# KevinLADLee/RoboRTS-Edu-SLAM

Hardware: AMD Instinct MI355X
Metric: candidate-pose scorings/sec (1081-beam scan, 2000×2000 grid) at 1/2/4/8 GPUs (higher is better)
Workload: dtype f64; 1 GPU; config2: 1081-beam scans vs 2000x2000 @5cm fp32 grid, full 3-level coarse->fine->super-fine (sim-YAML windows 5070+1331+189 candidates/scan); levels=headline, scans_per_gpu=4096, parallelism=replicas x1 (scan-sharded, no collective)

## Files before the change

roborts-edu-slam_amd/csrc/csm_api.cpp:

```cpp
#include "csm_source_digest.h"
#include "csm_host.hpp"
#include "libm_sincos.hpp"

using namespace csmh;

extern "C" {

int csm_abi_version(void) { return CSM_ABI_VERSION; }

const char* csm_build_digest(void) { return CSM_SOURCE_DIGEST; }

int csm_create(int device, csm_ctx** out) {
  const char* lr = std::getenv("LOCAL_RANK");
  const char* lw = std::getenv("LOCAL_WORLD_SIZE");
  const int world = lw ? std::max(1, std::atoi(lw)) : 1;
  const int rank = (lr && world > 1) ? std::min(std::max(0, std::atoi(lr)), world - 1) : 0;
  return create_context(device, rank, world, out);
}

int csm_get_host_plan(csm_ctx* c, csm_host_plan* out) {
  if (!c || !out) return CSM_ERR_INVALID_ARG;
  *out = c->host_plan;
  return CSM_OK;
}
// ... 17 lines not shown
    return CSM_ERR_HIP;
  }
  context_host_plan(device, local_rank, local_world, &c->host_plan);
  if (const char* env = std::getenv("CSM_HOST_THREADS")) {
    const int v = std::atoi(env);
    if (v > 0) c->host_plan.threads = v;
  }
  c->host_threads = c->host_plan.threads;
  if (const char* env = std::getenv("CSM_FIRST_WINDOWS")) c->first_windows = c->first_windows_submit = std::max(0, std::atoi(env));
  if (const char* env = std::getenv("CSM_FIRST_WINDOWS_SUBMIT")) c->first_windows_submit = std::max(0, std::atoi(env));
  if (const char* env = std::getenv("CSM_SPLIT_HANDOFF_MIN")) c->split_handoff_min = std::max(2, std::atoi(env));
  if (const char* env = std::getenv("CSM_DEFER_HANDOFF")) c->defer_last_handoff = std::atoi(env) != 0;
  if (const char* env = std::getenv("CSM_HOST_SIGNAL")) c->host_signal = std::atoi(env) != 0;
  if (const char* env = std::getenv("CSM_FINISH")) {
    c->device_finish = std::strcmp(env, "host") != 0;
    c->fast_finish = std::strcmp(env, "exact") != 0;
  }
  if (const char* env = std::getenv("CSM_KERNEL")) {
    c->row_kernel = std::strcmp(env, "v2") != 0;
    c->box_kernel = std::strcmp(env, "v6") == 0 || std::strcmp(env, "v7") == 0;
    c->box_kernel = c->box_kernel || std::strcmp(env, "v8") == 0;
    c->phase_kernel = std::strcmp(env, "v7") == 0 || std::strcmp(env, "v8") == 0;
    c->tiny_kernel = std::strcmp(env, "v8") == 0;
    c->pair_kernel = false;
  }
  if (const char* env = std::getenv("CSM_PHASE_STRIPS")) c->phase_strips = std::atoi(env) != 0;
  if (const char* env = std::getenv("CSM_BG_RUNS")) c->bg_runs = std::max(0, std::min(std::atoi(env), 3));
  if (const char* env = std::getenv("CSM_PHASE_MARGIN_LOG2"))
    c->phase_margin_log2 = std::max(2, std::min(std::atoi(env), 20));
  if (const char* env = std::getenv("CSM_PIPELINE")) {
    const int v = std::atoi(env);
    c->pipeline_min = v > 0 ? v : INT32_MAX;
  }
  if (const char* env = std::getenv("CSM_PIPELINE_PARTS"))
    c->pipeline_parts = std::max(2, std::min(std::atoi(env), csm_ctx::kMaxParts));
  if (const char* env = std::getenv("CSM_SKIP_DEAD_LISTS")) c->skip_dead_lists = std::atoi(env) != 0;
  if (const char* env = std::getenv("CSM_SMALL")) c->small_path = std::atoi(env) != 0;
  if (const char* env = std::getenv("CSM_LIST_REDUCE_MIN")) c->list_reduce_min = std::max<long long>(0, std::atoll(env));
  if (const char* env = std::getenv("CSM_STATS_DUMP")) c->stats_dump = std::atoi(env) != 0;
  if (const char* env = std::getenv("CSM_SCORE_MARKER")) c->score_marker = std::atoi(env) != 0;
  if (const char* env = std::getenv("CSM_DEVICE_TRIG")) c->device_trig = std::atoi(env) != 0;
#ifdef CSM_DEBUG_FIN
  c->debug_fin = true;
#endif
  if (c->each_slot([](LaunchSlot& s) { return s.create_sync_events(); }) != hipSuccess ||
      c->ev_pts.create(hipEventDisableTiming) != hipSuccess || c->ev_pack.create(hipEventDisableTiming) != hipSuccess ||
      c->x_stream.create(hipStreamNonBlocking) != hipSuccess) {
    delete c;
    return CSM_ERR_HIP;
  }
  {
    hipError_t we = c->h_pts.ensure((size_t)64 << 10);
    if (we == hipSuccess) we = c->pts.ensure((size_t)64 << 10);
    for (hipStream_t st : std::initializer_list<hipStream_t>{c->stream, c->h2d, c->d2h}) {
      if (we != hipSuccess) break;
      std::memset(c->h_pts.p, 0, (size_t)64 << 10);
      we = hipMemcpyAsync(c->pts.p, c->h_pts.p, (size_t)64 << 10, hipMemcpyHostToDevice, st);
      if (we == hipSuccess) we = hipMemcpyAsync(c->h_pts.p, c->pts.p, (size_t)64 << 10, hipMemcpyDeviceToHost, st);
      if (we == hipSuccess) we = hipStreamSynchronize(st);
    }
    if (we != hipSuccess) {
      csm_destroy(c);
      return CSM_ERR_HIP;
    }
  }
  *out = c;
  if (c->stats_dump) csm_set_profiling(c, 1);
  return CSM_OK;
// ... 251 lines not shown
```

roborts-edu-slam_amd/csrc/csm_driver.cpp:

```cpp
#include "csm_driver_internal.hpp"

using namespace csmh;

namespace {

struct BorrowedBatch {
  csm_ctx* c;
  ScanBatch* b;
  BorrowedBatch(csm_ctx* cc, ScanBatch* bb) : c(cc), b(bb) {
    if (b) c->swap_batch(*b);
  }
  ~BorrowedBatch() {
    if (b) c->swap_batch(*b);
  }
  BorrowedBatch(const BorrowedBatch&) = delete;
  BorrowedBatch& operator=(const BorrowedBatch&) = delete;
};

}

int csmh::matchers_loaded_locked(csm_ctx* c, const csm_param all_levels[3], int32_t use_fine, double* poses,
                                 double* covs, double* scores, int32_t first_level, const double* score_seed) {
  if (c->n_scans < 0) return c->fail(CSM_ERR_INVALID_ARG, "no scans loaded (csm_load_scans)");
  if (!c->has_grid) return c->fail(CSM_ERR_NO_GRID, "no grid set");
  const int32_t n_scans = c->n_scans;
  if (n_scans == 0) return CSM_OK;
  const double t_call = now_ms();
  c->t_call = t_call;
  if (c->profiling && c->t_exit > 0.0) c->account("host:between_calls", (float)(t_call - c->t_exit), 0.0, 0.0);
  std::vector<double> resp((size_t)n_scans, 0.0), sum((size_t)n_scans, 0.0);
  if (score_seed) sum.assign(score_seed, score_seed + n_scans);
  const csm_param* levels = all_levels + first_level;
  const int n_levels = use_fine ? 3 - first_level : 1;
// ... 46 lines not shown
  return match_level(c, n_scans, off.data(), *param, poses, covs, responses, argmax_flat);
}

int csm_scan_match(csm_ctx* c, const double* pts, int32_t n_points, const csm_param* param,
                   double pose[3], double cov[9], double* response, int64_t* argmax_flat) {
  if (!c || !response) return CSM_ERR_INVALID_ARG;
  const int64_t off[2] = {0, n_points < 0 ? 0 : n_points};
  if (n_points < 0) return c->fail(CSM_ERR_INVALID_ARG, "negative point count");
  return csm_scan_match_batch(c, 1, pts, off, param, pose, cov, response, argmax_flat);
}

int csm_scan_matchers_submit(csm_ctx* c, const csm_param levels[3], int32_t use_fine, double* poses, double* covs,
                             double* scores) {
  if (!c || !levels || !poses || !covs || !scores) return CSM_ERR_INVALID_ARG;
  std::lock_guard<std::mutex> lk(c->mu);
  DeviceGuard g(c->device);
  int st;
  if (c->staged_count == 0 && c->n_scans < 0) return c->fail(CSM_ERR_INVALID_ARG, "no scans loaded (csm_load_scans)");
  if (!c->has_grid) return c->fail(CSM_ERR_NO_GRID, "no grid set");
  ScanBatch* parked = nullptr;
  if (c->staged_count > 0) {
    parked = &c->staged[c->staged_head].batch;
    if ((st = take_staged(c)) != CSM_OK) return st;
  }
  auto prior_last_launches = [&]() {
    BorrowedBatch own(c, parked);
    return pipe_last_launches(c);
  };
  const int32_t n_scans = c->n_scans;
  const int n_levels = use_fine ? 3 : 1;
  bool fast = false;
  for (int l = 0; l < n_levels; ++l) fast |= levels[l].type == CSM_FAST;
  const int32_t* grid = c->scan_grid.empty() ? nullptr : c->scan_grid.data();
  const int K = std::max(2, std::min(c->pipeline_parts, csm_ctx::kMaxParts));
  if (n_scans == 0 || fast || grid || n_scans < c->pipeline_min || 2 * K > csm_ctx::kMaxParts) {
    if ((st = prior_last_launches()) != CSM_OK || (st = pipe_drain(c)) != CSM_OK) return st;
    return matchers_loaded_locked(c, levels, use_fine, poses, covs, scores);
  }
  const double t_call = now_ms();
  c->t_call = t_call;
  PipeState& PS = pipe_of(c);
  PipeJob& J = PS.job[PS.next];
  PipeJob& P = PS.job[PS.next ^ 1];
  if (J.pending && ((st = prior_last_launches()) != CSM_OK || (st = pipe_drain(c)) != CSM_OK))
    return st;
  PipeMode mode(c);
  job_setup(c, J, n_scans, c->scan_off.data(), levels, n_levels, poses, covs, nullptr, nullptr, K, PS.next * K,
            true);
  J.own_sum.assign((size_t)n_scans, 0.0);
  J.sum = J.own_sum.data();
  J.scores = scores;
  if ((st = job_begin(c, J, 0)) != CSM_OK) return pipe_abort(c, st);
  if ((st = prior_last_launches()) != CSM_OK) return pipe_abort(c, st);
  for (int h = 1; h < K; ++h)
    if ((st = job_begin(c, J, h)) != CSM_OK) return pipe_abort(c, st);
  if (P.pending && (st = job_finish(c, P)) != CSM_OK) return pipe_abort(c, st);
  if ((st = job_levels(c, J)) != CSM_OK) return pipe_abort(c, st);
  PS.next ^= 1;
  if (c->profiling) {
    c->t_exit = now_ms();
    c->account("host:submit", (float)(c->t_exit - t_call), 0.0, 0.0);
  }
  return CSM_OK;
}

int csm_scan_matchers_wait(csm_ctx* c) {
  if (!c) return CSM_ERR_INVALID_ARG;
  std::lock_guard<std::mutex> lk(c->mu);
  DeviceGuard g(c->device);
  return pipe_drain(c);
}

int csm_scan_matchers_loaded(csm_ctx* c, const csm_param levels[3], int32_t use_fine, double* poses,
                             double* covs, double* scores) {
  if (!c || !levels || !poses || !covs || !scores) return CSM_ERR_INVALID_ARG;
  std::lock_guard<std::mutex> lk(c->mu);
  DeviceGuard g(c->device);
  int st0;
  if ((st0 = pipe_drain(c)) != CSM_OK || (st0 = take_staged(c)) != CSM_OK) return st0;
  return matchers_loaded_locked(c, levels, use_fine, poses, covs, scores);
}

int csm_scan_matchers_batch(csm_ctx* c, int32_t n_scans, const double* pts, const int64_t* offsets,
                            const csm_param levels[3], int32_t use_fine, double* poses, double* covs,
                            double* scores) {
  if (!c || !levels || !poses || !covs || !scores) return CSM_ERR_INVALID_ARG;
  std::lock_guard<std::mutex> lk(c->mu);
  DeviceGuard g(c->device);
  const int st = load_scans_locked(c, n_scans, pts, offsets);
  if (st != CSM_OK) return st;
// ... 40 lines not shown
```

roborts-edu-slam_amd/csrc/csm_driver_internal.hpp:

```cpp
#pragma once

#include "csm_host.hpp"

namespace csmh {

struct LevelRun {
  csm_param P{};
  Dims D;
  std::vector<int> scan_of;
  std::vector<WindowPlan> plans;
  std::vector<int64_t> pt_off;
  std::vector<int32_t> grid;
  const AngleEntry* angles = nullptr;
  AngleEntry* rows = nullptr;
  const csm::FinishOut* fin = nullptr;
  const double* scores = nullptr;
  bool dev = false;
  int skip_lists = 0;
  PendingRun pend;
  int tag = -1;
  std::vector<csm::FinishOut>* snap = nullptr;
  std::vector<char>* how = nullptr;
  mutable int err = 0;
  const int32_t* order = nullptr;
// ... 26 lines not shown
    sw = nullptr;
    sw_stride = 0;
    int_bad = 0;
    int_known = false;
    shape = LevelSummary{};
    range_preset = false;
    dev_trig = false;
    trig_bad = 0;
  }
};

struct PipeJob {
  int K = 2, n_levels = 0, slot0 = 0;
  int first_windows = 0;
  int32_t n_scans = 0;
  const int64_t* offsets = nullptr;
  const int32_t* scan_grid = nullptr;
  csm_param levels[3]{};
  double *poses = nullptr, *covs = nullptr, *sum = nullptr;
  double* scores = nullptr;
  std::vector<double> resp, own_sum;
  int32_t first[csm_ctx::kMaxParts]{}, count[csm_ctx::kMaxParts]{};
  LevelRun R[2][csm_ctx::kMaxParts];
  bool pending = false;
  bool last_handoff_done = false;
  std::vector<int32_t> order[csm_ctx::kMaxParts];
  std::vector<csm::FinishOut> snaps[csm_ctx::kMaxParts];
  std::vector<char> hows[csm_ctx::kMaxParts];
};

struct PipeState {
  PipeJob job[2];
  int next = 0;
};

struct PipeMode {
  csm_ctx* c;
  bool small_was;
  explicit PipeMode(csm_ctx* cc) : c(cc), small_was(cc->small_path) {
    c->small_path = false;
    c->early_now = true;
  }
  ~PipeMode() {
    c->small_path = small_was;
    c->early_now = false;
  }
};

int live_lists(const csm_param* levels, int n_levels, int l);
int level_begin(csm_ctx* c, int32_t n_scans, const int64_t* offsets, const csm_param& P, const double* poses,
                double* responses, int64_t* argmax_flat, LevelRun& R, const int32_t* scan_grid, int skip_lists);
int level_begin_split(csm_ctx* c, int32_t n_scans, const int64_t* offsets, const csm_param& P, const double* poses,
                      double* responses, LevelRun& R, const int32_t* scan_grid, int skip_lists, int first);
int level_end(csm_ctx* c, LevelRun& R, double* poses, double* covs, double* responses, int64_t* argmax_flat);
int level_end_begin(csm_ctx* c, LevelRun& R, LevelRun& N, int32_t n_scans, const int64_t* offsets,
                    const csm_param& P, double* poses, double* covs, double* responses, double* sum,
                    const int32_t* scan_grid, int skip_lists, bool split = false);

PipeState& pipe_of(csm_ctx* c);
void job_setup(csm_ctx* c, PipeJob& J, int32_t n_scans, const int64_t* offsets, const csm_param* levels,
               int n_levels, double* poses, double* covs, double* sum, const int32_t* scan_grid, int K, int slot0,
               bool submitted = false);
int job_begin(csm_ctx* c, PipeJob& J, int h);
int job_levels(csm_ctx* c, PipeJob& J);
int job_finish(csm_ctx* c, PipeJob& J);
int pipe_abort(csm_ctx* c, int st);
int pipe_last_launches(csm_ctx* c);
int match_levels_pipelined(csm_ctx* c, int32_t n_scans, const int64_t* offsets, const csm_param* levels,
                           int n_levels, double* poses, double* covs, double* sum,
                           const int32_t* scan_grid = nullptr);

}
```

roborts-edu-slam_amd/csrc/csm_host.hpp:

```cpp
#pragma once

#include "csm.h"
#include "csm_internal.hpp"
#include "csm_finish_rules.hpp"
#include "csm_gridmap.h"
#include "csm_gridmap_internal.hpp"
#include "csm_resources.hpp"
#include "host_math.hpp"
#include "csm_pyramid.hpp"
#include "csm_search_match.hpp"
#include "csm_level_decision.hpp"
#include "csm_grid_copies.hpp"

#include <algorithm>
#include <atomic>
#include <chrono>
#include <condition_variable>
#include <functional>
#include <memory>
#include <cfloat>
#include <cmath>
#include <cstdio>
#include <cstdlib>
#include <cstring>
// ... 214 lines not shown
    }
  }
  int n_threads_;
  csm_host_plan plan_;
  static constexpr int chunk_div_ = 8;
  std::vector<std::thread> workers_;
  std::mutex mu_;
  std::condition_variable cv_;
  const std::function<void(int)>* job_ = nullptr;
  int n_items_ = 0, wanted_ = 0, chunk_ = 1;
  std::atomic<uint64_t> epoch_{0};
  std::atomic<uint64_t> claim_{0};
  std::atomic<int> done_{0};
  bool stop_ = false;
  int64_t start_ns_ = 0;
  std::atomic<int64_t> first_join_ns_{0}, last_join_ns_{0}, busy_ns_{0};
  double last_caller_share_ = 0.0, last_join_us_ = -1.0, last_last_join_us_ = -1.0, last_wall_us_ = 0.0,
         last_busy_us_ = 0.0;
};

inline double now_ms() {
  return std::chrono::duration<double, std::milli>(std::chrono::steady_clock::now().time_since_epoch()).count();
}


struct PendingRun {
  char kname[48] = {0};
  char fname[48] = {0};
  double alg_bytes = 0.0, scorings = 0.0, finish_bytes = 0.0;
  bool device_finish = false, timed = false;
  hipEvent_t ev0 = nullptr, ev1 = nullptr, ev2 = nullptr, done = nullptr;
  hipEvent_t ev_fast = nullptr;
  hipEvent_t gap0 = nullptr, gap1 = nullptr;
  const int32_t* flags = nullptr;
  int n_flags = 0;
  const csm::FinishOut* fin_host = nullptr;
  const int32_t* host_flag = nullptr;
  int32_t flag_value = 0;
  const int32_t* fast_flag = nullptr;
  bool defer_timing = false;
};

struct CtxStreams {
  Stream stream;
  Stream h2d, d2h;
  Stream x_stream;
  Stream stage_stream;
};

struct LaunchSlot {
  DevBuf scans, angles, scores, partials, best, fin;
  DevBuf ang_max;
  DevBuf win_ctr;
  HostBuf h_scores, h_fin, h_angles, h_sw;
  HostBuf h_angles_next;
  DevBuf fin_sig;
  HostBuf h_fin_sig;
  Event ev0, ev1, ev2;
  Event ev_ft;
  Event ev_g0, ev_g1;
  Event ev_done;
  Event ev_in;
  Event ev_k;
  Event ev_fast;
  bool span_gap = false;
  int32_t list_tag = 0;
  bool tail_open = false;

  hipError_t create_sync_events() {
    hipError_t e = hipSuccess;
    for (Event* ev : {&ev_done, &ev_in, &ev_k, &ev_fast})
      if (e == hipSuccess) e = ev->create(hipEventDisableTiming);
    return e;
  }
  hipError_t create_timing_events() {
    hipError_t e = hipSuccess;
    for (Event* ev : {&ev0, &ev1, &ev2, &ev_ft, &ev_g0, &ev_g1})
      if (e == hipSuccess) e = ev->create(hipEventDefault);
    return e;
  }
};

struct GridState {
  csm_map_info info{};
  bool has_grid = false;
  const float* d_grid = nullptr;
  DevBuf grid_buf;
  DevBuf gridi;
  const int32_t* d_gridi = nullptr;
  const void* key_cells = nullptr;
  int64_t key_stride = 0, key_version = -1;
  int32_t key_sx = -1, key_sy = -1;
  bool int_checked = false, int_ok = false;
  int int_exp = 0;
  int32_t pitch = 0;
  int32_t n_grids = 1;
  int32_t outside_i = 0;
  double int_max_abs = 0.0;
// ... 117 lines not shown
  Staged staged[2];
  int staged_head = 0, staged_count = 0;
  void swap_batch(csmh::ScanBatch& b) {
    std::swap(static_cast<csmh::ScanBatch&>(*this), b);
    pts_cached = b.pts_cached = false;
  }
  csmh::DevBuf laser_tab;
  bool laser_tab_ready = false;
  int32_t laser_tab_beams = 0;
  uint32_t laser_tab_amin = 0, laser_tab_ainc = 0;
  csmh::DevBuf deskew_tab;
  std::vector<double> deskew_tab_host;
  bool deskew_tab_ready = false;
  int32_t deskew_tab_beams = 0;
  uint32_t deskew_tab_amin = 0, deskew_tab_ainc = 0;

  bool profiling = false;
  bool profile_first_level = false;
  bool stats_dump = false;

  static constexpr int kMaxParts = 4;
  csmh::LaunchSlot alt[kMaxParts - 1];
  template <class F>
  hipError_t each_slot(F&& fn) {
    hipError_t e = fn(static_cast<csmh::LaunchSlot&>(*this));
    for (auto& a : alt)
      if (e == hipSuccess) e = fn(a);
    return e;
  }
  int pipeline_min = 512;
  bool skip_dead_lists = true;
  int64_t list_reduce_min = 8192;
  int pipeline_parts = 2;
  int first_windows = 128;
  int first_windows_submit = 512;
  int first_windows_submit_min_use = 512;
  int span_growth = 4;
  void* pipe = nullptr;
  bool split_last_handoff = true;
  int split_handoff_min = 256;
  bool defer_last_handoff = true;
  int part0_permille = 550;
  int part0_permille_submit = 500;
  void swap_slot(int i) {
    std::swap(static_cast<csmh::LaunchSlot&>(*this), alt[i - 1]);
  }
  void account_pool(const char* what) {
    if (!profiling || !pool) return;
    char nm[48];
    std::snprintf(nm, sizeof(nm), "pool:%s", what);
    account(nm, (float)(std::max(0.0, pool->last_join_us()) * 1e-3), pool->last_caller_share(), 0.0);
    std::snprintf(nm, sizeof(nm), "pool:%s:wall", what);
    account(nm, (float)(pool->last_wall_us() * 1e-3), std::max(0.0, pool->last_last_join_us()), pool->last_busy_us());
  }
  std::vector<csmh::PendingRun> deferred;
  std::vector<csm_kernel_stat> stats;
  void account_count(const char* name, int64_t n) {
    account(name, 0.0f, 0.0, 0.0);
    for (auto& s : stats)
      if (std::strncmp(s.name, name, sizeof(s.name)) == 0) s.launches += n - 1;
  }
  void account(const char* name, float ms, double bytes, double scorings) {
    for (auto& s : stats)
      if (std::strncmp(s.name, name, sizeof(s.name)) == 0) {
        s.launches += 1;
        s.total_ms += ms;
// ... 138 lines not shown
```

roborts-edu-slam_amd/csrc/csm_launch.cpp:

```cpp
#include "csm_host.hpp"
#include "libm_sincos_table.hpp"

namespace csmh {

int window_dims(const csm_param& P, Dims& d) {
  if (!(P.search_angle_resolution > 0.0) || !(P.search_space_resolution > 0.0) ||
      !(P.search_angle_offset >= 0.0) || !(P.search_space_size >= 0.0))
    return CSM_ERR_INVALID_ARG;
  const double half = (P.search_angle_offset * 2) / 2;
  const double na = std::floor(half * 2 / P.search_angle_resolution) + 1;
  const double ns = round_half_away(P.search_space_size / P.search_space_resolution) + 1;
  if (!(na >= 1.0 && na < 1e7 && ns >= 1.0 && ns < 1e7)) return CSM_ERR_INVALID_ARG;
  d.n_angles = (int32_t)na;
  d.n_space = (int32_t)ns;
  d.n_cand = (int64_t)d.n_angles * d.n_space * d.n_space;
  return CSM_OK;
}

bool beam_rule(int n, int use_point_size, int& step, int& use, int& n_used) {
  use = use_point_size;
  if (n < 2 * use) {
    use = n;
    step = 1;
  } else {
// ... 34 lines not shown
    }
    if (p.timed && (e = hipEventSynchronize(p.done)) != hipSuccess) return c->hip_fail(e, "hipEventSynchronize");
  } else if ((e = hipEventSynchronize(p.done)) != hipSuccess) {
    return c->hip_fail(e, "hipEventSynchronize");
  }
  return account_run(c, p);
}

int flush_deferred(csm_ctx* c) {
  int st = CSM_OK;
  for (const PendingRun& p : c->deferred) {
    const hipError_t e = hipEventSynchronize(p.done);
    if (e != hipSuccess) {
      st = c->hip_fail(e, "hipEventSynchronize(deferred)");
      break;
    }
    if ((st = account_run(c, p)) != CSM_OK) break;
  }
  c->deferred.clear();
  return st;
}

int account_run(csm_ctx* c, const PendingRun& p) {
  hipError_t e;
  if (p.timed) {
    float ms = 0.f;
    if ((e = hipEventElapsedTime(&ms, p.ev0, p.ev1)) != hipSuccess) return c->hip_fail(e, "hipEventElapsedTime");
    if (p.gap0) {
      float g = 0.f;
      if ((e = hipEventElapsedTime(&g, p.gap0, p.gap1)) != hipSuccess) return c->hip_fail(e, "hipEventElapsedTime");
      ms -= g;
    }
    c->account(p.kname, ms, p.alg_bytes, p.scorings);
    if (p.gap0) {
      char nm[48];
      std::snprintf(nm, sizeof(nm), "span2:%.41s", p.kname);
      c->account(nm, ms, p.alg_bytes, 0.0);
    }
    if (p.device_finish) {
      if ((e = hipEventElapsedTime(&ms, p.ev1, p.ev2)) != hipSuccess) return c->hip_fail(e, "hipEventElapsedTime");
      c->account(p.fname, ms, p.finish_bytes, 0.0);
      if (p.ev_fast) {
        float mf = 0.f, mx = 0.f;
        if ((e = hipEventElapsedTime(&mf, p.ev1, p.ev_fast)) != hipSuccess ||
            (e = hipEventElapsedTime(&mx, p.ev_fast, p.ev2)) != hipSuccess)
          return c->hip_fail(e, "hipEventElapsedTime");
        const char* lt = std::strchr(p.fname, '<');
        char nm[48];
        std::snprintf(nm, sizeof(nm), "finish:fast%s", lt ? lt : "");
        c->account(nm, mf, 0.0, 0.0);
        std::snprintf(nm, sizeof(nm), "finish:exact%s", lt ? lt : "");
        c->account(nm, mx, 0.0, 0.0);
      }
      if (p.flags) {
        int exact = 0;
        for (int i = 0; i < p.n_flags; ++i) exact += p.flags[i] != 0;
        c->account("finish:exact_windows", 0.f, 0.0, (double)exact);
        char nm[48];
        const char* lt = std::strchr(p.fname, '<');
        std::snprintf(nm, sizeof(nm), "finish:exact_windows%s", lt ? lt : "");
        c->account(nm, 0.f, (double)p.n_flags, (double)exact);
      }
    }
  }
  return CSM_OK;
}

bool phase_table(double f, int ns, int margin_log2, csm::PhaseTable& T) {
  T = csm::PhaseTable{};
  if (!(f > 0.0 && f < 1.0) || ns < 1 || ns > csm::kPhaseMaxSpace) return false;
// ... 493 lines not shown
    case ScoreKernel::kBoxPair:
      return csm::launch_score_box_pair(L, d_sw, d_pts, d_ang, d_out, d_partials, s.n_space, stream);
    case ScoreKernel::kBox: return csm::launch_score_box(L, d_sw, d_pts, d_ang, d_out, d_partials, s.n_space, stream);
    case ScoreKernel::kBoxTiled: return csm::launch_score_box(L, d_sw, d_pts, d_ang, d_out, d_partials, 16, stream);
    case ScoreKernel::kPhase:
      return csm::launch_score_phase(L, PT, d_sw, d_pts, d_ang, d_out, d_partials, s.n_space, stream);
    case ScoreKernel::kTiny: return csm::launch_score_tiny(L, d_sw, d_pts, d_ang, d_out, d_partials, s.n_space, stream);
    case ScoreKernel::kRows:
      return csm::launch_score_rows(L, d_sw, d_pts, d_ang, d_out, d_partials, s.n_space, s.rows_sq, stream);
    case ScoreKernel::kCols: return csm::launch_score_cols(L, d_sw, d_pts, d_ang, d_out, d_partials, s.kt, stream);
  }
  return hipErrorInvalidValue;
}

int Launch::scoring() {
  const bool best = mode == Finish::kBest;
  hipError_t e;
  if (sp.score && c->score_marker && !(c->profiling && w0 == 0) &&
      (e = hipEventRecord(c->ev_k, c->stream)) != hipSuccess)
    return c->hip_fail(e, "hipEventRecord");
  if (c->profiling && sp.score && w0 == 0 && (e = hipEventRecord(c->ev0, c->stream)) != hipSuccess)
    return c->hip_fail(e, "hipEventRecord");
  if (c->profiling && sp.score && w0 > 0 && !c->span_gap) {
    if ((e = hipEventRecord(c->ev_g1, c->stream)) != hipSuccess) return c->hip_fail(e, "hipEventRecord");
    c->span_gap = true;
  }
  if (best) {
    if ((e = c->partials.ensure((size_t)nw * (size_t)shape.bps * sizeof(BestPartial))) != hipSuccess)
      return c->hip_fail(e, "hipMalloc(partials)");
    if ((e = c->best.ensure((size_t)nw * sizeof(BestPartial))) != hipSuccess) return c->hip_fail(e, "hipMalloc(best)");
  } else if ((e = c->scores.ensure((size_t)nw * (size_t)stride * sizeof(double))) != hipSuccess) {
    return c->hip_fail(e, "hipMalloc(scores)");
  }
  if (sp.score &&
      (e = launch_score(shape, L, PT, (const ScanWork*)c->scans.p + w0, (const double*)c->pts.p,
                        (const AngleEntry*)c->angles.p, best ? nullptr : (double*)c->scores.p,
                        best ? (BestPartial*)c->partials.p : nullptr, c->stream)) != hipSuccess)
    return c->hip_fail(e, best ? "score kernel (best)" : "score kernel");
  if (dec.tail && sp.score) c->tail_open = w1 < nw;
  if (sp.score && c->profiling && (e = hipEventRecord(c->ev1, c->stream)) != hipSuccess)
    return c->hip_fail(e, "hipEventRecord");
  if (sp.score && !sp.finish && w0 == 0 && c->profiling && (e = hipEventRecord(c->ev_g0, c->stream)) != hipSuccess)
    return c->hip_fail(e, "hipEventRecord");
  return CSM_OK;
}

int Launch::finish_scores_to_host() {
  const size_t bytes = (size_t)nw * (size_t)D.n_cand * sizeof(double);
  hipError_t e;
  if ((e = c->h_scores.ensure(bytes)) != hipSuccess) return c->hip_fail(e, "hipHostMalloc(scores)");
  if ((e = hipEventRecord(c->ev_k, c->stream)) != hipSuccess || (e = hipStreamWaitEvent(c->d2h, c->ev_k, 0)) != hipSuccess)
    return c->hip_fail(e, "kernels event");
  if ((e = hipMemcpyAsync(c->h_scores.p, c->scores.p, bytes, hipMemcpyDeviceToHost, c->d2h)) != hipSuccess)
    return c->hip_fail(e, "hipMemcpyAsync(scores)");
  return CSM_OK;
}

int Launch::launch_finish_timed(const csm::FinishArgs& A, csm::FinishOut* out, hipStream_t fs, bool fast_done) {
  hipError_t e;
  if ((e = csm::launch_finish(A, (const ScanWork*)c->scans.p, (const AngleEntry*)c->angles.p,
                              (const double*)c->scores.p, out, nw, c->stream, fs, c->ev_fast, fast_done)) != hipSuccess)
    return c->hip_fail(e, "finish_kernel");
  if (time_fin() && fs != c->stream && (e = hipEventRecord(c->ev_ft, c->stream)) != hipSuccess)
    return c->hip_fail(e, "hipEventRecord");
  if (time_fin() && (e = hipEventRecord(c->ev2, fs)) != hipSuccess) return c->hip_fail(e, "hipEventRecord");
  return CSM_OK;
// ... 34 lines not shown
  const BestPartial* parts = (const BestPartial*)c->partials.p;
  hipError_t e;
  if (shape.kernel == ScoreKernel::kBoxTiled) {
    const int32_t tpw = shape.ktiles * shape.ktiles;
    if ((e = c->best_tiles.ensure((size_t)nw * tpw * sizeof(BestPartial))) != hipSuccess)
      return c->hip_fail(e, "hipMalloc(tile bests)");
    if ((e = csm::launch_reduce_best(parts, D.n_angles, nw * tpw, (BestPartial*)c->best_tiles.p, c->stream)) !=
            hipSuccess ||
        (e = csm::launch_reduce_best((const BestPartial*)c->best_tiles.p, tpw, nw, (BestPartial*)c->best.p,
                                     c->stream)) != hipSuccess)
      return c->hip_fail(e, "reduce_best_kernel");
  } else if ((e = csm::launch_reduce_best(parts, (int32_t)shape.bps, nw, (BestPartial*)c->best.p, c->stream)) !=
             hipSuccess) {
    return c->hip_fail(e, "reduce_best_kernel");
  }
  if ((e = hipEventRecord(c->ev_k, c->stream)) != hipSuccess || (e = hipStreamWaitEvent(c->d2h, c->ev_k, 0)) != hipSuccess)
    return c->hip_fail(e, "kernels event");
  if ((e = hipMemcpyAsync(best_out, c->best.p, (size_t)nw * sizeof(BestPartial), hipMemcpyDeviceToHost, c->d2h)) != hipSuccess)
    return c->hip_fail(e, "hipMemcpyAsync(best)");
  return CSM_OK;
}

void Launch::fill_pending(const char* kname, PendingRun& p) {
  pending_base(c, D, plans, kname, p);
  p.flags = flags_h;
  p.n_flags = n_flags;
  p.device_finish = mode == Finish::kDevice && time_fin();
  p.ev_fast = (time_fin() && mode == Finish::kDevice && c->fast_finish && c->x_stream) ? (hipEvent_t)c->ev_ft : nullptr;
  if (c->span_gap) {
    p.gap0 = c->ev_g0;
    p.gap1 = c->ev_g1;
    c->span_gap = false;
  }
  p.fin_host = sig_out;
  p.host_flag = SA.host_flag;
  p.fast_flag = SA.host_fast_flag;
  p.flag_value = SA.flag_value;
  p.defer_timing = sig;
}

int run_windows(csm_ctx* c, const csm_param& P, const Dims& D, const Geometry& G,
                const std::vector<WindowPlan>& plans, const std::vector<int64_t>& pt_offsets,
                const AngleEntry* angles, size_t n_angle_entries,
                const std::vector<int32_t>& grid_index, BestPartial* best_out,
                Finish mode, PendingRun* pend, int skip_lists, WinSpan sp) {
  if (best_out) mode = Finish::kBest;
  const int nw = (int)plans.size();
  if (nw == 0) return CSM_OK;
  const int w0 = sp.w1 < 0 ? 0 : sp.w0, w1 = sp.w1 < 0 ? nw : sp.w1;
  Launch X{c,  P,  D,  G,  plans, angles, n_angle_entries, mode, skip_lists,
           sp, nw, w0, w1, w0 == 0 && w1 == nw && sp.score && sp.finish, P.search_space_resolution / G.mres};
  const double tp0 = c->profiling ? now_ms() : 0.0;
  if (!c->deferred.empty()) {
    const int fst = flush_deferred(c);
    if (fst != CSM_OK) return fst;
  }
  const double tp1 = c->profiling ? now_ms() : 0.0;
  if (c->profiling) c->account("host:launch:flush_events", (float)(tp1 - tp0), 0.0, 0.0);
  int st;
  hipError_t e;
  if ((st = X.validate()) != CSM_OK) return st;
  if (X.whole && mode != Finish::kBest && c->int_ok && X.S.in_range && small_launch(c, D, nw))
    return run_windows_small(c, P, D, G, plans, pt_offsets, angles, n_angle_entries, grid_index,
                             mode == Finish::kDevice, pend, skip_lists);
  if ((st = X.decide()) != CSM_OK) return st;
  if ((st = X.level_work(pt_offsets, grid_index)) != CSM_OK) return st;
// ... 156 lines not shown
```

roborts-edu-slam_amd/csrc/csm_pipeline.cpp:

```cpp
#include "csm_driver_internal.hpp"

namespace csmh {
namespace {

template <typename F>
int with_slot(csm_ctx* c, const PipeJob& J, int h, F&& f) {
  const int sidx = J.slot0 + h;
  if (sidx > 0) c->swap_slot(sidx);
  const int st = f();
  if (sidx > 0) c->swap_slot(sidx);
  return st;
}

#ifndef CSM_WINDOW_ORDER
#define CSM_WINDOW_ORDER 1
#endif
void window_order(const Geometry& G, const double* poses, int32_t n, std::vector<int32_t>& out) {
  out.resize((size_t)n);
  thread_local std::vector<uint32_t> key, key2;
  thread_local std::vector<int32_t> idx2;
  key.resize((size_t)n);
  key2.resize((size_t)n);
  idx2.resize((size_t)n);
  auto spread = [](uint32_t v) {
    v &= 0xFFFF;
    v = (v | (v << 8)) & 0x00FF00FFu;
    v = (v | (v << 4)) & 0x0F0F0F0Fu;
    v = (v | (v << 2)) & 0x33333333u;
    v = (v | (v << 1)) & 0x55555555u;
    return v;
  };
  for (int32_t s = 0; s < n; ++s) {
    double m[3];
    G.to_map(poses + 3 * (size_t)s, m);
    const double qx = std::floor(m[0] / 64.0), qy = std::floor(m[1] / 64.0);
    const uint32_t ix = (uint32_t)((int32_t)std::max(-32768.0, std::min(32767.0, qx)) + 32768);
    const uint32_t iy = (uint32_t)((int32_t)std::max(-32768.0, std::min(32767.0, qy)) + 32768);
    key[(size_t)s] = spread(ix) | (spread(iy) << 1);
  }
  std::vector<int32_t>& idx = out;
  for (int32_t s = 0; s < n; ++s) idx[(size_t)s] = s;
  for (int shift = 0; shift < 32; shift += 8) {
    size_t cnt[257] = {0};
    for (int32_t i = 0; i < n; ++i) ++cnt[((key[(size_t)i] >> shift) & 0xFF) + 1];
    for (int d = 0; d < 256; ++d) cnt[d + 1] += cnt[d];
    for (int32_t i = 0; i < n; ++i) {
      const size_t o = cnt[(key[(size_t)i] >> shift) & 0xFF]++;
      key2[o] = key[(size_t)i];
      idx2[o] = idx[(size_t)i];
    }
    key.swap(key2);
    idx.swap(idx2);
  }
  if (CSM_WINDOW_ORDER == 2) return;
  idx2.assign(idx.begin(), idx.end());
  int32_t pos = 0;
  for (int x = 0; x < 8; ++x)
    for (int32_t m = x; m < n; m += 8) out[(size_t)pos++] = idx2[(size_t)m];
}

int job_skip(const csm_ctx* c, const PipeJob& J, int l) {
  return c->skip_dead_lists ? live_lists(J.levels, J.n_levels, l) : 0;
}

int job_handoff(csm_ctx* c, PipeJob& J, int l, int h) {
  const int32_t s0 = J.first[h];
  J.R[(l + 1) & 1][h].tag = (l + 1) * 8 + h;
  const bool timed = c->profiling;
  c->profiling = timed && !c->profile_first_level;
  const int st = with_slot(c, J, h, [&] {
    return level_end_begin(c, J.R[l & 1][h], J.R[(l + 1) & 1][h], J.count[h], J.offsets + s0, J.levels[l + 1],
                           J.poses + 3 * (size_t)s0, J.covs + 9 * (size_t)s0, J.resp.data() + s0, J.sum + s0,
                           J.scan_grid ? J.scan_grid + s0 : nullptr, job_skip(c, J, l + 1),
                           c->split_last_handoff && h == J.K - 1 && l + 2 == J.n_levels);
  });
  c->profiling = timed;
  return st;
}

int job_last_handoff(csm_ctx* c, PipeJob& J) {
  if (!J.pending || J.last_handoff_done) return CSM_OK;
  J.last_handoff_done = true;
  return job_handoff(c, J, J.n_levels - 2, J.K - 1);
}

}

PipeState& pipe_of(csm_ctx* c) {
  if (!c->pipe) c->pipe = new PipeState();
  return *static_cast<PipeState*>(c->pipe);
}

void job_setup(csm_ctx* c, PipeJob& J, int32_t n_scans, const int64_t* offsets, const csm_param* levels,
               int n_levels, double* poses, double* covs, double* sum, const int32_t* scan_grid, int K, int slot0,
               bool submitted) {
  J.K = K;
  J.first_windows = !submitted ? c->first_windows
                    : (n_levels > 0 && levels[0].use_point_size > c->first_windows_submit_min_use) ? c->first_windows_submit
                                                                                                   : 0;
  const int permille = submitted ? c->part0_permille_submit : c->part0_permille;
  J.n_levels = n_levels;
  J.slot0 = slot0;
  J.n_scans = n_scans;
  J.offsets = offsets;
  J.scan_grid = scan_grid;
  for (int l = 0; l < n_levels; ++l) J.levels[l] = levels[l];
  J.poses = poses;
  J.covs = covs;
  J.sum = sum;
  J.scores = nullptr;
  J.pending = false;
  J.last_handoff_done = false;
  const int64_t n0 = (K == 2 && permille > 0) ? (int64_t)n_scans * permille / 1000
                                                        : (int64_t)n_scans / K;
  for (int h = 0; h < K; ++h) {
    J.first[h] = h == 0 ? 0 : (int32_t)(n0 + (int64_t)(n_scans - n0) * (h - 1) / (K - 1));
    J.count[h] = (h == 0 ? (int32_t)n0 : (int32_t)(n0 + (int64_t)(n_scans - n0) * h / (K - 1))) - J.first[h];
  }
  J.resp.assign((size_t)n_scans, 0.0);
  for (auto& row : J.R)
    for (LevelRun& r : row) r.reset();
  for (int h = 0; h < K; ++h) J.order[h].clear();
}

int job_begin(csm_ctx* c, PipeJob& J, int h) {
  const int32_t s0 = J.first[h];
  J.R[0][h].tag = h;
  if (CSM_WINDOW_ORDER) {
    window_order(Geometry(c->info), J.poses + 3 * (size_t)s0, J.count[h], J.order[h]);
    J.R[0][h].order = J.R[1][h].order = J.order[h].data();
  }
  return with_slot(c, J, h, [&] {
    const int32_t* g = J.scan_grid ? J.scan_grid + s0 : nullptr;
    if (h == 0)
      return level_begin_split(c, J.count[h], J.offsets + s0, J.levels[0], J.poses + 3 * (size_t)s0,
                               J.resp.data() + s0, J.R[0][h], g, job_skip(c, J, 0), J.first_windows);
    return level_begin(c, J.count[h], J.offsets + s0, J.levels[0], J.poses + 3 * (size_t)s0, J.resp.data() + s0,
                       nullptr, J.R[0][h], g, job_skip(c, J, 0));
  });
}

int job_levels(csm_ctx* c, PipeJob& J) {
  const int K = J.K, n_levels = J.n_levels;
  int st;
  for (int l = 0; l + 1 < n_levels; ++l)
    for (int h = 0; h < K; ++h) {
      if (c->defer_last_handoff && l + 2 == n_levels && h == K - 1) continue;
      if ((st = job_handoff(c, J, l, h)) != CSM_OK) return st;
    }
  J.pending = true;
  J.last_handoff_done = n_levels < 2 || !c->defer_last_handoff;
  return CSM_OK;
}

int job_finish(csm_ctx* c, PipeJob& J) {
  if (!J.pending) return CSM_OK;
  int st;
  if ((st = job_last_handoff(c, J)) != CSM_OK) return st;
  J.pending = false;
  const int K = J.K, last = J.n_levels - 1;
  for (int h = 0; h < K; ++h) {
    const int32_t s0 = J.first[h];
    LevelRun& cur = J.R[last & 1][h];
    if (c->debug_fin) {
      J.snaps[h].assign(cur.scan_of.size(), csm::FinishOut{});
      J.hows[h].assign(cur.scan_of.size(), (char)3);
      cur.snap = &J.snaps[h];
      cur.how = &J.hows[h];
    }
    if ((st = level_end(c, cur, J.poses + 3 * (size_t)s0, J.covs + 9 * (size_t)s0, J.resp.data() + s0, nullptr)) !=
        CSM_OK)
      return st;
    for (int s = s0; s < s0 + J.count[h]; ++s) J.sum[(size_t)s] += J.resp[(size_t)s];
  }
  if (J.scores)
    for (int s = 0; s < J.n_scans; ++s) J.scores[s] = J.sum[(size_t)s] / J.n_levels;
  if (c->debug_fin) {
    (void)hipDeviceSynchronize();
    for (int h = 0; h < K; ++h) {
      const LevelRun& L = J.R[last & 1][h];
      if (!L.dev || !L.fin) continue;
      for (size_t i = 0; i < J.snaps[h].size(); ++i) {
        const csm::FinishOut& a = J.snaps[h][i];
        const csm::FinishOut& b = L.fin[i];
        const int lists = (int)(b.seal_tag_kind >> 34) & 3;
// ... 73 lines not shown
```

Before: 13.89 billion scorings/s.

## Submit unsplit single-part job when coarse level is device-bound

Adds a submit-order planner that picks the number of pipeline parts per submitted job. When the coarse level is device-bound and no part count was set, it uses one part instead of two. With one part, the first handoff is issued before the prior job's finish to keep the device fed. Slot indexing now uses a fixed half-capacity, and the profiler records dispatch counts. The trade is fewer, larger launches and less intra-job overlap against lower per-part launch and sync overhead.

```diff
diff --git a/roborts-edu-slam_amd/csrc/csm_api.cpp b/roborts-edu-slam_amd/csrc/csm_api.cpp
--- a/roborts-edu-slam_amd/csrc/csm_api.cpp
+++ b/roborts-edu-slam_amd/csrc/csm_api.cpp
@@ -73,8 +73,12 @@
     const int v = std::atoi(env);
     c->pipeline_min = v > 0 ? v : INT32_MAX;
   }
-  if (const char* env = std::getenv("CSM_PIPELINE_PARTS"))
+  if (const char* env = std::getenv("CSM_PIPELINE_PARTS")) {
     c->pipeline_parts = std::max(2, std::min(std::atoi(env), csm_ctx::kMaxParts));
+    c->pipeline_parts_set = true;
+  }
+  if (const char* env = std::getenv("CSM_SUBMIT_PARTS")) c->submit_parts = std::max(0, std::min(std::atoi(env), 2));
+  if (const char* env = std::getenv("CSM_SINGLE_SPLIT_HANDOFF")) c->single_split_handoff = std::atoi(env) != 0;
   if (const char* env = std::getenv("CSM_SKIP_DEAD_LISTS")) c->skip_dead_lists = std::atoi(env) != 0;
   if (const char* env = std::getenv("CSM_SMALL")) c->small_path = std::atoi(env) != 0;
   if (const char* env = std::getenv("CSM_LIST_REDUCE_MIN")) c->list_reduce_min = std::max<long long>(0, std::atoll(env));
diff --git a/roborts-edu-slam_amd/csrc/csm_driver.cpp b/roborts-edu-slam_amd/csrc/csm_driver.cpp
--- a/roborts-edu-slam_amd/csrc/csm_driver.cpp
+++ b/roborts-edu-slam_amd/csrc/csm_driver.cpp
@@ -1,4 +1,5 @@
 #include "csm_driver_internal.hpp"
+#include "csm_submit_order.hpp"
 
 using namespace csmh;
 
@@ -111,8 +112,9 @@
   bool fast = false;
   for (int l = 0; l < n_levels; ++l) fast |= levels[l].type == CSM_FAST;
   const int32_t* grid = c->scan_grid.empty() ? nullptr : c->scan_grid.data();
-  const int K = std::max(2, std::min(c->pipeline_parts, csm_ctx::kMaxParts));
-  if (n_scans == 0 || fast || grid || n_scans < c->pipeline_min || 2 * K > csm_ctx::kMaxParts) {
+  const int K = submit_parts(c->submit_parts, c->pipeline_parts_set, std::min(c->pipeline_parts, csm_ctx::kMaxParts),
+                             coarse_device_bound(c, levels, n_levels));
+  if (n_scans == 0 || fast || grid || n_scans < c->pipeline_min || K > PipeState::kParts) {
     if ((st = prior_last_launches()) != CSM_OK || (st = pipe_drain(c)) != CSM_OK) return st;
     return matchers_loaded_locked(c, levels, use_fine, poses, covs, scores);
   }
@@ -124,17 +126,23 @@
   if (J.pending && ((st = prior_last_launches()) != CSM_OK || (st = pipe_drain(c)) != CSM_OK))
     return st;
   PipeMode mode(c);
-  job_setup(c, J, n_scans, c->scan_off.data(), levels, n_levels, poses, covs, nullptr, nullptr, K, PS.next * K,
-            true);
+  job_setup(c, J, n_scans, c->scan_off.data(), levels, n_levels, poses, covs, nullptr, nullptr, K,
+            PS.next * PipeState::kParts, true);
   J.own_sum.assign((size_t)n_scans, 0.0);
   J.sum = J.own_sum.data();
   J.scores = scores;
-  if ((st = job_begin(c, J, 0)) != CSM_OK) return pipe_abort(c, st);
-  if ((st = prior_last_launches()) != CSM_OK) return pipe_abort(c, st);
-  for (int h = 1; h < K; ++h)
-    if ((st = job_begin(c, J, h)) != CSM_OK) return pipe_abort(c, st);
-  if (P.pending && (st = job_finish(c, P)) != CSM_OK) return pipe_abort(c, st);
-  if ((st = job_levels(c, J)) != CSM_OK) return pipe_abort(c, st);
+  const SubmitOrder order = submit_order(K, P.pending ? P.K : 0, n_levels, c->defer_last_handoff);
+  for (int i = 0; i < order.n; ++i) {
+    const SubmitOp& op = order.op[i];
+    switch (op.step) {
+      case SubmitStep::kBegin: st = job_begin(c, J, op.part); break;
+      case SubmitStep::kHandoff: st = job_handoff(c, J, op.level, op.part); break;
+      case SubmitStep::kPriorLast: st = prior_last_launches(); break;
+      case SubmitStep::kPriorFinish: st = job_finish(c, P); break;
+    }
+    if (st != CSM_OK) return pipe_abort(c, st);
+  }
+  job_launched(c, J);
   PS.next ^= 1;
   if (c->profiling) {
     c->t_exit = now_ms();
diff --git a/roborts-edu-slam_amd/csrc/csm_driver_internal.hpp b/roborts-edu-slam_amd/csrc/csm_driver_internal.hpp
--- a/roborts-edu-slam_amd/csrc/csm_driver_internal.hpp
+++ b/roborts-edu-slam_amd/csrc/csm_driver_internal.hpp
@@ -82,6 +82,7 @@
 struct PipeState {
   PipeJob job[2];
   int next = 0;
+  static constexpr int kParts = csm_ctx::kMaxParts / 2;
 };
 
 struct PipeMode {
@@ -96,6 +97,10 @@
     c->early_now = false;
   }
 };
+
+inline bool coarse_device_bound(const csm_ctx* c, const csm_param* levels, int n_levels) {
+  return n_levels > 0 && levels[0].use_point_size > c->first_windows_submit_min_use;
+}
 
 int live_lists(const csm_param* levels, int n_levels, int l);
 int level_begin(csm_ctx* c, int32_t n_scans, const int64_t* offsets, const csm_param& P, const double* poses,
@@ -112,7 +117,9 @@
                int n_levels, double* poses, double* covs, double* sum, const int32_t* scan_grid, int K, int slot0,
                bool submitted = false);
 int job_begin(csm_ctx* c, PipeJob& J, int h);
+int job_handoff(csm_ctx* c, PipeJob& J, int l, int h);
 int job_levels(csm_ctx* c, PipeJob& J);
+void job_launched(const csm_ctx* c, PipeJob& J);
 int job_finish(csm_ctx* c, PipeJob& J);
 int pipe_abort(csm_ctx* c, int st);
 int pipe_last_launches(csm_ctx* c);
diff --git a/roborts-edu-slam_amd/csrc/csm_host.hpp b/roborts-edu-slam_amd/csrc/csm_host.hpp
--- a/roborts-edu-slam_amd/csrc/csm_host.hpp
+++ b/roborts-edu-slam_amd/csrc/csm_host.hpp
@@ -270,6 +270,7 @@
   hipEvent_t ev0 = nullptr, ev1 = nullptr, ev2 = nullptr, done = nullptr;
   hipEvent_t ev_fast = nullptr;
   hipEvent_t gap0 = nullptr, gap1 = nullptr;
+  int dispatches = 1;
   const int32_t* flags = nullptr;
   int n_flags = 0;
   const csm::FinishOut* fin_host = nullptr;
@@ -302,6 +303,7 @@
   Event ev_k;
   Event ev_fast;
   bool span_gap = false;
+  int span_count = 0;
   int32_t list_tag = 0;
   bool tail_open = false;
 
@@ -485,6 +487,9 @@
   bool skip_dead_lists = true;
   int64_t list_reduce_min = 8192;
   int pipeline_parts = 2;
+  bool pipeline_parts_set = false;
+  int submit_parts = 0;
+  bool single_split_handoff = false;
   int first_windows = 128;
   int first_windows_submit = 512;
   int first_windows_submit_min_use = 512;
diff --git a/roborts-edu-slam_amd/csrc/csm_launch.cpp b/roborts-edu-slam_amd/csrc/csm_launch.cpp
--- a/roborts-edu-slam_amd/csrc/csm_launch.cpp
+++ b/roborts-edu-slam_amd/csrc/csm_launch.cpp
@@ -90,10 +90,12 @@
       ms -= g;
     }
     c->account(p.kname, ms, p.alg_bytes, p.scorings);
+    if (p.dispatches > 1) c->account_count(p.kname, p.dispatches - 1);
     if (p.gap0) {
       char nm[48];
       std::snprintf(nm, sizeof(nm), "span2:%.41s", p.kname);
       c->account(nm, ms, p.alg_bytes, 0.0);
+      if (p.dispatches > 1) c->account_count(nm, p.dispatches - 1);
     }
     if (p.device_finish) {
       if ((e = hipEventElapsedTime(&ms, p.ev1, p.ev2)) != hipSuccess) return c->hip_fail(e, "hipEventElapsedTime");
@@ -653,6 +655,7 @@
   } else if ((e = c->scores.ensure((size_t)nw * (size_t)stride * sizeof(double))) != hipSuccess) {
     return c->hip_fail(e, "hipMalloc(scores)");
   }
+  if (sp.score) c->span_count = w0 == 0 ? 1 : c->span_count + 1;
   if (sp.score &&
       (e = launch_score(shape, L, PT, (const ScanWork*)c->scans.p + w0, (const double*)c->pts.p,
                         (const AngleEntry*)c->angles.p, best ? nullptr : (double*)c->scores.p,
@@ -753,6 +756,8 @@
     p.gap1 = c->ev_g1;
     c->span_gap = false;
   }
+  p.dispatches = std::max(1, c->span_count);
+  c->span_count = 0;
   p.fin_host = sig_out;
   p.host_flag = SA.host_flag;
   p.fast_flag = SA.host_fast_flag;
diff --git a/roborts-edu-slam_amd/csrc/csm_pipeline.cpp b/roborts-edu-slam_amd/csrc/csm_pipeline.cpp
--- a/roborts-edu-slam_amd/csrc/csm_pipeline.cpp
+++ b/roborts-edu-slam_amd/csrc/csm_pipeline.cpp
@@ -1,4 +1,5 @@
 #include "csm_driver_internal.hpp"
+#include "csm_submit_order.hpp"
 
 namespace csmh {
 namespace {
@@ -63,41 +64,40 @@
   return c->skip_dead_lists ? live_lists(J.levels, J.n_levels, l) : 0;
 }
 
+}
+
+PipeState& pipe_of(csm_ctx* c) {
+  if (!c->pipe) c->pipe = new PipeState();
+  return *static_cast<PipeState*>(c->pipe);
+}
+
 int job_handoff(csm_ctx* c, PipeJob& J, int l, int h) {
   const int32_t s0 = J.first[h];
   J.R[(l + 1) & 1][h].tag = (l + 1) * 8 + h;
   const bool timed = c->profiling;
   c->profiling = timed && !c->profile_first_level;
+  const bool split = (J.K > 1 ? c->split_last_handoff : c->single_split_handoff) && h == J.K - 1 && l + 2 == J.n_levels;
   const int st = with_slot(c, J, h, [&] {
     return level_end_begin(c, J.R[l & 1][h], J.R[(l + 1) & 1][h], J.count[h], J.offsets + s0, J.levels[l + 1],
                            J.poses + 3 * (size_t)s0, J.covs + 9 * (size_t)s0, J.resp.data() + s0, J.sum + s0,
                            J.scan_grid ? J.scan_grid + s0 : nullptr, job_skip(c, J, l + 1),
-                           c->split_last_handoff && h == J.K - 1 && l + 2 == J.n_levels);
+                           split);
   });
   c->profiling = timed;
   return st;
 }
 
-int job_last_handoff(csm_ctx* c, PipeJob& J) {
+static int job_last_handoff(csm_ctx* c, PipeJob& J) {
   if (!J.pending || J.last_handoff_done) return CSM_OK;
   J.last_handoff_done = true;
   return job_handoff(c, J, J.n_levels - 2, J.K - 1);
-}
-
-}
-
-PipeState& pipe_of(csm_ctx* c) {
-  if (!c->pipe) c->pipe = new PipeState();
-  return *static_cast<PipeState*>(c->pipe);
 }
 
 void job_setup(csm_ctx* c, PipeJob& J, int32_t n_scans, const int64_t* offsets, const csm_param* levels,
                int n_levels, double* poses, double* covs, double* sum, const int32_t* scan_grid, int K, int slot0,
                bool submitted) {
   J.K = K;
-  J.first_windows = !submitted ? c->first_windows
-                    : (n_levels > 0 && levels[0].use_point_size > c->first_windows_submit_min_use) ? c->first_windows_submit
-                                                                                                   : 0;
+  J.first_windows = !submitted ? c->first_windows : coarse_device_bound(c, levels, n_levels) ? c->first_windows_submit : 0;
   const int permille = submitted ? c->part0_permille_submit : c->part0_permille;
   J.n_levels = n_levels;
   J.slot0 = slot0;
@@ -113,9 +113,11 @@
   J.last_handoff_done = false;
   const int64_t n0 = (K == 2 && permille > 0) ? (int64_t)n_scans * permille / 1000
                                                         : (int64_t)n_scans / K;
-  for (int h = 0; h < K; ++h) {
-    J.first[h] = h == 0 ? 0 : (int32_t)(n0 + (int64_t)(n_scans - n0) * (h - 1) / (K - 1));
-    J.count[h] = (h == 0 ? (int32_t)n0 : (int32_t)(n0 + (int64_t)(n_scans - n0) * h / (K - 1))) - J.first[h];
+  J.first[0] = 0;
+  J.count[0] = (int32_t)n0;
+  for (int h = 1; h < K; ++h) {
+    J.first[h] = (int32_t)(n0 + (int64_t)(n_scans - n0) * (h - 1) / (K - 1));
+    J.count[h] = (int32_t)(n0 + (int64_t)(n_scans - n0) * h / (K - 1)) - J.first[h];
   }
   J.resp.assign((size_t)n_scans, 0.0);
   for (auto& row : J.R)
@@ -145,12 +147,16 @@
   int st;
   for (int l = 0; l + 1 < n_levels; ++l)
     for (int h = 0; h < K; ++h) {
-      if (c->defer_last_handoff && l + 2 == n_levels && h == K - 1) continue;
+      if (handoff_deferred(l, h, K, n_levels, c->defer_last_handoff)) continue;
       if ((st = job_handoff(c, J, l, h)) != CSM_OK) return st;
     }
+  job_launched(c, J);
+  return CSM_OK;
+}
+
+void job_launched(const csm_ctx* c, PipeJob& J) {
   J.pending = true;
-  J.last_handoff_done = n_levels < 2 || !c->defer_last_handoff;
-  return CSM_OK;
+  J.last_handoff_done = J.n_levels < 2 || !c->defer_last_handoff;
 }
 
 int job_finish(csm_ctx* c, PipeJob& J) {
diff --git a/roborts-edu-slam_amd/csrc/csm_submit_order.hpp b/roborts-edu-slam_amd/csrc/csm_submit_order.hpp
--- /dev/null
+++ b/roborts-edu-slam_amd/csrc/csm_submit_order.hpp
@@ -0,0 +1,53 @@
+#pragma once
+
+namespace csmh {
+
+constexpr bool handoff_deferred(int l, int h, int parts, int levels, bool defer) {
+  return defer && l + 2 == levels && h == parts - 1;
+}
+
+enum class SubmitStep : unsigned char {
+  kBegin,
+  kHandoff,
+  kPriorLast,
+  kPriorFinish,
+};
+
+struct SubmitOp {
+  SubmitStep step;
+  int level, part;
+  constexpr bool operator==(const SubmitOp& o) const { return step == o.step && level == o.level && part == o.part; }
+};
+
+constexpr int kSubmitMaxParts = 4;
+constexpr int kSubmitMaxLevels = 3;
+
+struct SubmitOrder {
+  SubmitOp op[kSubmitMaxParts * kSubmitMaxLevels + 2]{};
+  int n = 0;
+  constexpr void add(SubmitStep s, int level = 0, int part = 0) { op[n++] = SubmitOp{s, level, part}; }
+};
+
+constexpr SubmitOrder submit_order(int parts, int pending_parts, int levels, bool defer) {
+  SubmitOrder o;
+  o.add(SubmitStep::kBegin, 0, 0);
+  if (pending_parts > 0) o.add(SubmitStep::kPriorLast);
+  for (int h = 1; h < parts; ++h) o.add(SubmitStep::kBegin, 0, h);
+  const bool early_handoff = parts == 1 && levels > 1 && !handoff_deferred(0, 0, parts, levels, defer);
+  if (early_handoff) o.add(SubmitStep::kHandoff, 0, 0);
+  if (pending_parts > 0) o.add(SubmitStep::kPriorFinish);
+  for (int l = 0; l + 1 < levels; ++l)
+    for (int h = 0; h < parts; ++h) {
+      if (handoff_deferred(l, h, parts, levels, defer) || (early_handoff && l == 0)) continue;
+      o.add(SubmitStep::kHandoff, l, h);
+    }
+  return o;
+}
+
+constexpr int submit_parts(int forced, bool pipeline_parts_set, int pipeline_parts, bool coarse_device_bound) {
+  if (forced == 1 || forced == 2) return forced;
+  if (pipeline_parts_set || !coarse_device_bound) return pipeline_parts < 2 ? 2 : pipeline_parts;
+  return 1;
+}
+
+}
```

Measured after the change: 14.72 billion scorings/s, median of 6. 1.06x the previous value.
